# RuyiLian/CheckerPose

Measured on AMD Instinct MI355X. Metric: crops/sec forward (256x256, npt=512), higher is better.
Workload: dtype bf16; 1 GPU; LMO 'ape' hr18GNN2_res6_gnn3Skip_mlpQuery npt=512, PoseNet_GNNskip forward, deterministic random-init weights; global_batch=256, parallelism=dp1 (no forward collective), launch=hipGraph replay of 104 kernel launches

## Files before the change

### checkerpose_amd/csrc/conv3x3_halo.hip

```cpp
#include <stdlib.h>

#include "common.h"
#include <cstring>

struct HaloParams {
  const void* in; const void* w; const float* scale; const float* shift; const void* res; void* out;
  int B, H, W, Cin, in_cs, in_coff, nchunk, Cout, ngroups, NB;
  int tiles_x, tiles_y, total_tiles;
  int act; float slope;
  uint32_t in_bytes, w_bytes;
  long long o_base, o_sb, o_sy, o_sx;
  int Hs, Ws; float up_sy, up_sx;
  const float* seg_w; const float* seg_b; float* seg_out; int seg_S;
};

constexpr int HTH = 8, HTW = 16, HPW = HTW + 2, HPH = HTH + 2, HNPIX = 192;
constexpr int HPLANE = HNPIX * 16, HBUF = 4 * HPLANE;
constexpr int USRH = 7, USRW = 11, USPIX = 80, USBUF = USPIX * 64;

template <typename Tag> struct MmaH;
template <> struct MmaH<F32Tag> {
  static __device__ __forceinline__ void run(const u32x4& w, const u32x4& a, f32x4& acc) {
    acc = __builtin_amdgcn_mfma_f32_16x16x4f32(__uint_as_float(w.x), __uint_as_float(a.x), acc, 0, 0, 0);
    acc = __builtin_amdgcn_mfma_f32_16x16x4f32(__uint_as_float(w.y), __uint_as_float(a.y), acc, 0, 0, 0);
    acc = __builtin_amdgcn_mfma_f32_16x16x4f32(__uint_as_float(w.z), __uint_as_float(a.z), acc, 0, 0, 0);
    acc = __builtin_amdgcn_mfma_f32_16x16x4f32(__uint_as_float(w.w), __uint_as_float(a.w), acc, 0, 0, 0);
  }
};
template <> struct MmaH<BF16Tag> {
  static __device__ __forceinline__ void run(const u32x4& w, const u32x4& a, f32x4& acc) {
    acc = __builtin_amdgcn_mfma_f32_16x16x32_bf16(__builtin_bit_cast(bf16x8, w), __builtin_bit_cast(bf16x8, a), acc, 0, 0, 0);
  }
};

template <typename Tag, bool HAS_RES>
__global__ __launch_bounds__(256) void conv3x3_halo_kernel(const HaloParams p) {
  constexpr int E = Tag::E;
  constexpr int KCH = 4 * E;
  constexpr int ES = 16 / E;
  extern __shared__ __attribute__((aligned(16))) unsigned char smem[];

  const int label = blockIdx.x & 7, slot = blockIdx.x >> 3;
  const int nblk = slot % p.NB;
  const int t = label * ((p.total_tiles + 7) >> 3) + slot / p.NB;
  if (t >= p.total_tiles) return;
  const int tpi = p.tiles_x * p.tiles_y;
  const int b = t / tpi;
  const int trem = t - b * tpi;
  const int ty = trem / p.tiles_x, tx = trem - ty * p.tiles_x;
  const int y0 = ty * HTH, x0 = tx * HTW;

  const int tid = threadIdx.x;
  const int lane = tid & 63;
  const int wave = __builtin_amdgcn_readfirstlane(tid >> 6);
  const int x = lane & 15, q = lane >> 4;
  const int g = nblk * 4 + wave;
  const bool wave_active = g < p.ngroups;

  const __amdgpu_buffer_rsrc_t rsrc = __builtin_amdgcn_make_buffer_rsrc(const_cast<void*>(p.in), 0, p.in_bytes, 0x00020000);
  const __amdgpu_buffer_rsrc_t wrsrc = __builtin_amdgcn_make_buffer_rsrc(const_cast<void*>(p.w), 0, p.w_bytes, 0x00020000);

  uint32_t s_goff[3];
  uint32_t s_lds[3];
  int s_cq[3];
#pragma unroll
  for (int k = 0; k < 3; ++k) {
    const int i = tid + 256 * k;
    const int hp = i >> 2, pq = i & 3;
    const int py = hp / HPW, px = hp - py * HPW;
    const int gy = y0 - 1 + py, gx = x0 - 1 + px;
    const bool ok = (hp < HPH * HPW) & ((unsigned)gy < (unsigned)p.H) & ((unsigned)gx < (unsigned)p.W);
    s_goff[k] = ok ? (uint32_t)(((b * p.H + gy) * p.W + gx) * p.in_cs + p.in_coff + pq * E) : 0xFFFFFFFFu;
    s_lds[k] = (uint32_t)(pq * HPLANE + (hp < HNPIX ? hp : 0) * 16);
    s_cq[k] = pq * E;
  }
  const bool s_do[3] = {true, true, (tid + 512) < HNPIX * 4};

  auto stage_load = [&](u32x4* v, int c) {
    const int c0 = c * KCH;
#pragma unroll
    for (int k = 0; k < 3; ++k) {
      const bool ok = (s_goff[k] != 0xFFFFFFFFu) & (c0 + s_cq[k] < p.Cin);
      const uint32_t off = ok ? (s_goff[k] + (uint32_t)c0) * ES : 0x80000000u;
      v[k] = __builtin_bit_cast(u32x4, __builtin_amdgcn_raw_buffer_load_b128(rsrc, off, 0, 0));
    }
  };
  auto stage_write = [&](const u32x4* v, int buf) {
#pragma unroll
    for (int k = 0; k < 3; ++k)
      if (s_do[k]) *(u32x4*)(smem + buf * HBUF + s_lds[k]) = v[k];
  };

  f32x4 acc[HTH][2];
#pragma unroll
  for (int mt = 0; mt < HTH; ++mt) { acc[mt][0] = f32x4{0.f, 0.f, 0.f, 0.f}; acc[mt][1] = f32x4{0.f, 0.f, 0.f, 0.f}; }

  const uint32_t wbase = ((uint32_t)(wave_active ? g : 0) * p.nchunk * 18u * 64u + lane) * 16u;
  auto w_load = [&](u32x4* w, int c, int tap) {
    const uint32_t off = wbase + ((uint32_t)c * 18u + (uint32_t)tap * 2u) * 1024u;
    w[0] = __builtin_bit_cast(u32x4, __builtin_amdgcn_raw_buffer_load_b128(wrsrc, off, 0, 0));
    w[1] = __builtin_bit_cast(u32x4, __builtin_amdgcn_raw_buffer_load_b128(wrsrc, off + 1024u, 0, 0));
  };
  const uint32_t a_lane = (uint32_t)(q * HPLANE + x * 16);
  auto a_load = [&](u32x4* a, int buf, int tap) {
    const int r = tap / 3, s = tap - 3 * r;
    const unsigned char* base = smem + buf * HBUF + a_lane + (r * HPW + s) * 16;
#pragma unroll
    for (int mt = 0; mt < HTH; ++mt) a[mt] = *(const u32x4*)(base + mt * HPW * 16);
  };
  auto mma = [&](const u32x4* a, const u32x4* w) {
#pragma unroll
    for (int mt = 0; mt < HTH; ++mt) {
      MmaH<Tag>::run(w[0], a[mt], acc[mt][0]);
      MmaH<Tag>::run(w[1], a[mt], acc[mt][1]);
    }
  };

  u32x4 sv[3];
  stage_load(sv, 0);
  u32x4 w0[2], w1[2], w2[2], aA[HTH], aB[HTH];
  w_load(w0, 0, 0);
  w_load(w1, 0, 1);
  stage_write(sv, 0);
  __syncthreads();

#define CP_TAP(T, ACUR, ANEXT, WCUR, WNEXT, CN, TN)                      \
  w_load(WNEXT, CN, TN);                                                 \
  if (T < 8) a_load(ANEXT, buf, T + 1);                                  \
  __builtin_amdgcn_sched_barrier(0);                                     \
  mma(ACUR, WCUR);                                                       \
  __builtin_amdgcn_sched_barrier(0);
  for (int c = 0; c < p.nchunk; ++c) {
    const int buf = c & 1;
    stage_load(sv, c + 1);
    a_load(aA, buf, 0);
    CP_TAP(0, aA, aB, w0, w2, c, 2)
    CP_TAP(1, aB, aA, w1, w0, c, 3)
    CP_TAP(2, aA, aB, w2, w1, c, 4)
    CP_TAP(3, aB, aA, w0, w2, c, 5)
    CP_TAP(4, aA, aB, w1, w0, c, 6)
    CP_TAP(5, aB, aA, w2, w1, c, 7)
    CP_TAP(6, aA, aB, w0, w2, c, 8)
    CP_TAP(7, aB, aA, w1, w0, c + 1, 0)
    CP_TAP(8, aA, aB, w2, w1, c + 1, 1)
    stage_write(sv, buf ^ 1);
    __syncthreads();
  }
#undef CP_TAP

  if (!wave_active) return;
  const int ch = g * 32 + q * 8;
  if (ch >= p.Cout) return;
  const bool hi_ok = ch + 4 < p.Cout;
  const int ox = x0 + x;
  float sc[8], sh[8];
  {
    const f32x4 s0 = *(const f32x4*)(p.scale + ch), t0 = *(const f32x4*)(p.shift + ch);
    const f32x4 s1 = *(const f32x4*)(p.scale + ch + 4), t1 = *(const f32x4*)(p.shift + ch + 4);
#pragma unroll
    for (int j = 0; j < 4; ++j) { sc[j] = s0[j]; sh[j] = t0[j]; sc[4 + j] = s1[j]; sh[4 + j] = t1[j]; }
  }
  if (ox >= p.W) return;
  float rvv[HAS_RES ? HTH : 1][8];
  if constexpr (HAS_RES) {
#pragma unroll
    for (int mt = 0; mt < HTH; ++mt) {
      const int oy = y0 + mt;
#pragma unroll
      for (int j = 0; j < 8; ++j) rvv[mt][j] = 0.f;
      if (oy >= p.H) continue;
      const long long o = p.o_base + (long long)b * p.o_sb + (long long)oy * p.o_sy + (long long)ox * p.o_sx + ch;
      if (E == 4) {
        const f32x4 r0 = *(const f32x4*)((const float*)p.res + o);
#pragma unroll
        for (int j = 0; j < 4; ++j) rvv[mt][j] = r0[j];
        if (hi_ok) {
          const f32x4 r1 = *(const f32x4*)((const float*)p.res + o + 4);
#pragma unroll
          for (int j = 0; j < 4; ++j) rvv[mt][4 + j] = r1[j];
        }
      } else {
        const u32x2 r0 = *(const u32x2*)((const uint16_t*)p.res + o);
        rvv[mt][0] = __uint_as_float(r0.x << 16); rvv[mt][1] = __uint_as_float(r0.x & 0xffff0000u);
        rvv[mt][2] = __uint_as_float(r0.y << 16); rvv[mt][3] = __uint_as_float(r0.y & 0xffff0000u);
        if (hi_ok) {
          const u32x2 r1 = *(const u32x2*)((const uint16_t*)p.res + o + 4);
          rvv[mt][4] = __uint_as_float(r1.x << 16); rvv[mt][5] = __uint_as_float(r1.x & 0xffff0000u);
          rvv[mt][6] = __uint_as_float(r1.y << 16); rvv[mt][7] = __uint_as_float(r1.y & 0xffff0000u);
        }
      }
    }
  }
#pragma unroll
  for (int mt = 0; mt < HTH; ++mt) {
    const int oy = y0 + mt;
    if (oy >= p.H) continue;
    const long long o = p.o_base + (long long)b * p.o_sb + (long long)oy * p.o_sy + (long long)ox * p.o_sx + ch;
    float v[8];
#pragma unroll
    for (int j = 0; j < 4; ++j) { v[j] = acc[mt][0][j] * sc[j] + sh[j]; v[4 + j] = acc[mt][1][j] * sc[4 + j] + sh[4 + j]; }
    if constexpr (HAS_RES) {
#pragma unroll
      for (int j = 0; j < 8; ++j) v[j] += rvv[HAS_RES ? mt : 0][j];
    }
#pragma unroll
    for (int j = 0; j < 8; ++j) {
      v[j] = cp_act_apply(v[j], cp_act_slope(p.act, p.slope));
    }
    if (E == 4) {
      *(f32x4*)((float*)p.out + o) = f32x4{v[0], v[1], v[2], v[3]};
      if (hi_ok) *(f32x4*)((float*)p.out + o + 4) = f32x4{v[4], v[5], v[6], v[7]};
    } else {
      if (hi_ok) {
        u32x4 pk; pk.x = pack_bf16x2(v[0], v[1]); pk.y = pack_bf16x2(v[2], v[3]); pk.z = pack_bf16x2(v[4], v[5]); pk.w = pack_bf16x2(v[6], v[7]);
        if ((((uintptr_t)((uint16_t*)p.out + o)) & 15u) == 0) *(u32x4*)((uint16_t*)p.out + o) = pk;
        else { *(u32x2*)((uint16_t*)p.out + o) = u32x2{pk.x, pk.y}; *(u32x2*)((uint16_t*)p.out + o + 4) = u32x2{pk.z, pk.w}; }
      } else {
        u32x2 pk; pk.x = pack_bf16x2(v[0], v[1]); pk.y = pack_bf16x2(v[2], v[3]);
        *(u32x2*)((uint16_t*)p.out + o) = pk;
      }
    }
  }
}


template <typename Tag, bool HAS_RES, bool UP = false, bool SEG = false>
__global__ __launch_bounds__(256, 2) void conv3x3_halo4_kernel(const HaloParams p) {
  constexpr int E = Tag::E;
  constexpr int KCH = 4 * E;
  constexpr int ES = 16 / E;
  extern __shared__ __attribute__((aligned(16))) unsigned char smem[];
  unsigned char* const sSrc = smem + 2 * HBUF;

  const int label = blockIdx.x & 7, slot = blockIdx.x >> 3;
  const int nblk = slot % p.NB;
  const int t = label * ((p.total_tiles + 7) >> 3) + slot / p.NB;
  if (t >= p.total_tiles) return;
  const int tpi = p.tiles_x * p.tiles_y;
  const int b = t / tpi;
  const int trem = t - b * tpi;
  const int ty = trem / p.tiles_x, tx = trem - ty * p.tiles_x;
  const int y0 = ty * HTH, x0 = tx * HTW;

  const int tid = threadIdx.x;
  const int lane = tid & 63;
  const int wave = __builtin_amdgcn_readfirstlane(tid >> 6);
  const int x = lane & 15, q = lane >> 4;
  const int g = nblk * 4 + wave;

  const __amdgpu_buffer_rsrc_t rsrc = __builtin_amdgcn_make_buffer_rsrc(const_cast<void*>(p.in), 0, p.in_bytes, 0x00020000);
  const __amdgpu_buffer_rsrc_t wrsrc = __builtin_amdgcn_make_buffer_rsrc(const_cast<void*>(p.w), 0, p.w_bytes, 0x00020000);

  uint32_t s_goff[3], s_lds[3];
  int s_cq[3];
#pragma unroll
  for (int k = 0; k < 3; ++k) {
    const int i = tid + 256 * k;
    const int hp = i >> 2, pq = i & 3;
    const int py = hp / HPW, px = hp - py * HPW;
    const int gy = y0 - 1 + py, gx = x0 - 1 + px;
    const bool ok = (hp < HPH * HPW) & ((unsigned)gy < (unsigned)p.H) & ((unsigned)gx < (unsigned)p.W);
    s_goff[k] = ok ? (uint32_t)(((b * p.H + gy) * p.W + gx) * p.in_cs + p.in_coff + pq * E) : 0xFFFFFFFFu;
    s_lds[k] = (uint32_t)(pq * HPLANE + hp * 16);
    s_cq[k] = pq * E;
  }
  auto stage_load = [&](u32x4* v, int c) {
    const int c0 = c * KCH;
#pragma unroll
    for (int k = 0; k < 3; ++k) {
      const bool ok = (s_goff[k] != 0xFFFFFFFFu) & (c0 + s_cq[k] < p.Cin);
      v[k] = __builtin_bit_cast(u32x4, __builtin_amdgcn_raw_buffer_load_b128(rsrc, ok ? (s_goff[k] + (uint32_t)c0) * ES : 0x80000000u, 0, 0));
    }
  };
  auto stage_write = [&](const u32x4* v, int buf) {
#pragma unroll
    for (int k = 0; k < 3; ++k) *(u32x4*)(smem + buf * HBUF + s_lds[k]) = v[k];
  };

  uint32_t u_goff[2], m_off[3];
  float m_lx[3], m_ly[3];
  if constexpr (UP) {
    int sy0, sx0, st_; float fr_;
    cp_up_coord(p.up_sy, y0 > 0 ? y0 - 1 : 0, p.Hs, sy0, st_, fr_);
    cp_up_coord(p.up_sx, x0 > 0 ? x0 - 1 : 0, p.Ws, sx0, st_, fr_);
#pragma unroll
    for (int k = 0; k < 2; ++k) {
      const int i = tid + 256 * k;
      const int sp = i >> 2, pq = i & 3;
      const int ry = sp / USRW, rx = sp - ry * USRW;
      const int yy = sy0 + ry, xx = sx0 + rx;
      const bool ok = (sp < USRH * USRW) & (yy < p.Hs) & (xx < p.Ws);
      u_goff[k] = ok ? (uint32_t)(((b * p.Hs + yy) * p.Ws + xx) * p.in_cs + p.in_coff + pq * E) : 0xFFFFFFFFu;
    }
#pragma unroll
    for (int k = 0; k < 3; ++k) {
      const int i = tid + 256 * k;
      const int hp = i >> 2, pq = i & 3;
      const int py = hp / HPW, px = hp - py * HPW;
      const int gy = y0 - 1 + py, gx = x0 - 1 + px;
      const bool ok = (hp < HPH * HPW) & ((unsigned)gy < (unsigned)p.H) & ((unsigned)gx < (unsigned)p.W);
      int iy0, ix0, my, mx;
      cp_up_coord(p.up_sy, gy, p.Hs, iy0, my, m_ly[k]);
      cp_up_coord(p.up_sx, gx, p.Ws, ix0, mx, m_lx[k]);
      m_off[k] = ok ? (uint32_t)((((iy0 - sy0) * USRW + (ix0 - sx0)) * 4 + pq) * 16) | (uint32_t)(mx | (my << 1) | 4) : 0u;
    }
  }
  auto src_load = [&](u32x4* v, int c) {
    const int c0 = c * KCH;
#pragma unroll
    for (int k = 0; k < 2; ++k) {
      const bool ok = (u_goff[k] != 0xFFFFFFFFu) & (c0 + (tid & 3) * E < p.Cin);
      v[k] = __builtin_bit_cast(u32x4, __builtin_amdgcn_raw_buffer_load_b128(rsrc, ok ? (u_goff[k] + (uint32_t)c0) * ES : 0x80000000u, 0, 0));
    }
  };
  auto src_write = [&](const u32x4* v, int sb) {
    *(u32x4*)(sSrc + sb * USBUF + tid * 16) = v[0];
    if (tid < USPIX * 4 - 256) *(u32x4*)(sSrc + sb * USBUF + (tid + 256) * 16) = v[1];
  };
  auto interp = [&](int k, int sb, int hb) {
    const uint32_t mo = m_off[k];
    const unsigned char* s00 = sSrc + sb * USBUF + (mo & ~15u);
    const uint32_t dx = (mo & 1u) ? 64u : 0u, dy = (mo & 2u) ? (uint32_t)(USRW * 64) : 0u;
    const float lx1 = m_lx[k], lx0 = cp_one_minus(lx1), ly1 = m_ly[k], ly0 = cp_one_minus(ly1);
    const bool in_img = (mo & 4u) != 0u;
    unsigned char* dst = smem + hb * HBUF + s_lds[k];
#pragma unroll
    for (int j = 0; j < 4; ++j) {
      const uint32_t r00 = *(const uint32_t*)(s00 + 4 * j), r01 = *(const uint32_t*)(s00 + dx + 4 * j);
      const uint32_t r10 = *(const uint32_t*)(s00 + dy + 4 * j), r11 = *(const uint32_t*)(s00 + dy + dx + 4 * j);
      uint32_t o;
      if constexpr (E == 4) {
        o = __float_as_uint(cp_bilerp(__uint_as_float(r00), __uint_as_float(r01), __uint_as_float(r10), __uint_as_float(r11), lx0, lx1, ly0, ly1));
      } else {
        const float lo = cp_bilerp(__uint_as_float(r00 << 16), __uint_as_float(r01 << 16), __uint_as_float(r10 << 16), __uint_as_float(r11 << 16), lx0, lx1, ly0, ly1);
        const float hi = cp_bilerp(__uint_as_float(r00 & 0xffff0000u), __uint_as_float(r01 & 0xffff0000u), __uint_as_float(r10 & 0xffff0000u),
                                   __uint_as_float(r11 & 0xffff0000u), lx0, lx1, ly0, ly1);
        o = pack_bf16x2(lo, hi);
      }
      *(uint32_t*)(dst + 4 * j) = in_img ? o : 0u;
    }
  };

  f32x4 acc[HTH][4];
#pragma unroll
  for (int mt = 0; mt < HTH; ++mt)
#pragma unroll
    for (int nt = 0; nt < 4; ++nt) acc[mt][nt] = f32x4{0.f, 0.f, 0.f, 0.f};

  const uint32_t wbase = ((uint32_t)g * p.nchunk * 36u * 64u + lane) * 16u;
  auto w_load = [&](u32x4* w, int c, int tap) {
    const uint32_t off = wbase + ((uint32_t)c * 36u + (uint32_t)tap * 4u) * 1024u;
#pragma unroll
    for (int nt = 0; nt < 4; ++nt) w[nt] = __builtin_bit_cast(u32x4, __builtin_amdgcn_raw_buffer_load_b128(wrsrc, off + nt * 1024u, 0, 0));
  };
  const uint32_t a_lane = (uint32_t)(q * HPLANE + x * 16);
  auto a_load = [&](u32x4* a, int buf, int tap, int half) {
    const int r = tap / 3, s2 = tap - 3 * r;
    const unsigned char* base = smem + buf * HBUF + a_lane + ((r + 4 * half) * HPW + s2) * 16;
#pragma unroll
    for (int i = 0; i < 4; ++i) a[i] = *(const u32x4*)(base + i * HPW * 16);
  };
  auto mma = [&](const u32x4* a, const u32x4* w, int half) {
#pragma unroll
    for (int i = 0; i < 4; ++i)
#pragma unroll
      for (int nt = 0; nt < 4; ++nt) MmaH<Tag>::run(w[nt], a[i], acc[4 * half + i][nt]);
  };

  u32x4 sv[3];
  u32x4 wA[4], wB[4], a0[4], a1[4];
  if constexpr (UP) {
    src_load(sv, 0);
    w_load(wA, 0, 0);
    src_write(sv, 0);
    src_load(sv, 1);
    __syncthreads();
    interp(0, 0, 0); interp(1, 0, 0); interp(2, 0, 0);
    src_write(sv, 1);
  } else {
    stage_load(sv, 0);
    w_load(wA, 0, 0);
    stage_write(sv, 0);
  }
  __syncthreads();

#define CP_TAP4(T, WCUR, WNEXT, CN, TN)                                                 \
  a_load(a1, buf, T, 1); w_load(WNEXT, CN, TN); __builtin_amdgcn_sched_barrier(0);       \
  mma(a0, WCUR, 0); __builtin_amdgcn_sched_barrier(0);                                   \
  if (T < 8) a_load(a0, buf, T + 1, 0);                                                  \
  __builtin_amdgcn_sched_barrier(0);                                                     \
  mma(a1, WCUR, 1); __builtin_amdgcn_sched_barrier(0);
  for (int c = 0; c < p.nchunk; ++c) {
    const int buf = c & 1;
    if constexpr (UP) src_load(sv, c + 2); else stage_load(sv, c + 1);
    a_load(a0, buf, 0, 0);
    CP_TAP4(0, wA, wB, c, 1)
    CP_TAP4(1, wB, wA, c, 2)
    if constexpr (UP) { __builtin_amdgcn_sched_barrier(0); interp(0, buf ^ 1, buf ^ 1); __builtin_amdgcn_sched_barrier(0); }
    CP_TAP4(2, wA, wB, c, 3)
    CP_TAP4(3, wB, wA, c, 4)
    CP_TAP4(4, wA, wB, c, 5)
    if constexpr (UP) { __builtin_amdgcn_sched_barrier(0); interp(1, buf ^ 1, buf ^ 1); __builtin_amdgcn_sched_barrier(0); }
    CP_TAP4(5, wB, wA, c, 6)
    CP_TAP4(6, wA, wB, c, 7)
    CP_TAP4(7, wB, wA, c, 8)
    if constexpr (UP) { __builtin_amdgcn_sched_barrier(0); interp(2, buf ^ 1, buf ^ 1); __builtin_amdgcn_sched_barrier(0); }
    CP_TAP4(8, wA, wB, c + 1, 0)
#pragma unroll
    for (int nt = 0; nt < 4; ++nt) wA[nt] = wB[nt];
    if constexpr (UP) src_write(sv, buf); else stage_write(sv, buf ^ 1);
    __syncthreads();
  }
#undef CP_TAP4

  const int ch = g * 64 + q * 16;
  const int ox = x0 + x;
  if constexpr (!SEG) { if (ox >= p.W) return; }
  const bool xok = SEG ? ox < p.W : true;
  constexpr int SMAX = 2;
  float segw[SEG ? SMAX : 1][16], segp[SEG ? 8 : 1][SEG ? SMAX : 1];
  if constexpr (SEG) {
#pragma unroll
    for (int s_ = 0; s_ < SMAX; ++s_) {
#pragma unroll
      for (int k = 0; k < 4; ++k) {
        const f32x4 w4 = s_ < p.seg_S ? *(const f32x4*)(p.seg_w + (size_t)s_ * p.Cout + ch + 4 * k) : f32x4{0.f, 0.f, 0.f, 0.f};
#pragma unroll
        for (int j = 0; j < 4; ++j) segw[s_][4 * k + j] = w4[j];
      }
#pragma unroll
      for (int mt = 0; mt < 8; ++mt) segp[mt][s_] = 0.f;
    }
  }
  float sc[16], sh[16];
#pragma unroll
  for (int nt = 0; nt < 4; ++nt) {
    const f32x4 s4 = *(const f32x4*)(p.scale + ch + 4 * nt), t4 = *(const f32x4*)(p.shift + ch + 4 * nt);
#pragma unroll
    for (int j = 0; j < 4; ++j) { sc[4 * nt + j] = s4[j]; sh[4 * nt + j] = t4[j]; }
  }
#pragma unroll
  for (int half = 0; half < 2; ++half) {
    u32x4 rr[HAS_RES ? 4 : 1][E == 4 ? 4 : 2];
    if constexpr (HAS_RES) {
#pragma unroll
      for (int i = 0; i < 4; ++i) {
        const int oy = y0 + 4 * half + i;
        const long long o = p.o_base + (long long)b * p.o_sb + (long long)oy * p.o_sy + (long long)ox * p.o_sx + ch;
#pragma unroll
        for (int k = 0; k < (E == 4 ? 4 : 2); ++k) {
          rr[i][k] = u32x4{0u, 0u, 0u, 0u};
          if (oy < p.H) rr[i][k] = E == 4 ? *(const u32x4*)((const float*)p.res + o + 4 * k) : *(const u32x4*)((const uint16_t*)p.res + o + 8 * k);
        }
      }
    }
#pragma unroll
    for (int i = 0; i < 4; ++i) {
      const int mt = 4 * half + i;
      const int oy = y0 + mt;
      if (oy >= p.H) continue;
      const long long o = p.o_base + (long long)b * p.o_sb + (long long)oy * p.o_sy + (long long)ox * p.o_sx + ch;
      float v[16];
#pragma unroll
      for (int nt = 0; nt < 4; ++nt)
#pragma unroll
        for (int j = 0; j < 4; ++j) v[4 * nt + j] = acc[mt][nt][j] * sc[4 * nt + j] + sh[4 * nt + j];
      if constexpr (HAS_RES) {
        if (E == 4) {
#pragma unroll
          for (int k = 0; k < 4; ++k) {
            v[4 * k + 0] += __uint_as_float(rr[i][k].x); v[4 * k + 1] += __uint_as_float(rr[i][k].y);
            v[4 * k + 2] += __uint_as_float(rr[i][k].z); v[4 * k + 3] += __uint_as_float(rr[i][k].w);
          }
        } else {
          float r8[8];
#pragma unroll
          for (int k = 0; k < 2; ++k) {
            Vec16<BF16Tag>::unpack(rr[i][k], r8);
#pragma unroll
            for (int j = 0; j < 8; ++j) v[8 * k + j] += r8[j];
          }
        }
      }
#pragma unroll
      for (int j = 0; j < 16; ++j) {
        v[j] = cp_act_apply(v[j], cp_act_slope(p.act, p.slope));
      }
      if (E == 4) {
        if (xok) {
#pragma unroll
          for (int k = 0; k < 4; ++k) *(f32x4*)((float*)p.out + o + 4 * k) = f32x4{v[4 * k], v[4 * k + 1], v[4 * k + 2], v[4 * k + 3]};
        }
      } else {
        const u32x4 pk0 = Vec16<BF16Tag>::pack(v), pk1 = Vec16<BF16Tag>::pack(v + 8);
        if (xok) {
          *(u32x4*)((uint16_t*)p.out + o) = pk0;
          *(u32x4*)((uint16_t*)p.out + o + 8) = pk1;
        }
        if constexpr (SEG) { Vec16<BF16Tag>::unpack(pk0, v); Vec16<BF16Tag>::unpack(pk1, v + 8); }
      }
      if constexpr (SEG) {
#pragma unroll
        for (int s_ = 0; s_ < SMAX; ++s_) {
          float a = 0.f;
#pragma unroll
          for (int j = 0; j < 16; ++j) a += v[j] * segw[s_][j];
          segp[mt][s_] = a;
        }
      }
    }
  }
  if constexpr (SEG) {
    float* const red = (float*)smem;
#pragma unroll
    for (int mt = 0; mt < 8; ++mt)
#pragma unroll
      for (int s_ = 0; s_ < SMAX; ++s_) {
        float a = segp[mt][s_];
        a += __shfl_xor(a, 16);
        a += __shfl_xor(a, 32);
        if (q == 0) red[((wave * 8 + mt) * 16 + x) * SMAX + s_] = a;
      }
    __syncthreads();
    const int s_ = tid & 1, px = tid >> 1;
    const int mt = px >> 4, xx = px & 15;
    const int oy = y0 + mt, oxx = x0 + xx;
    if (s_ < p.seg_S && oy < p.H && oxx < p.W) {
      float a = p.seg_b[s_];
#pragma unroll
      for (int wv = 0; wv < 4; ++wv) a += red[((wv * 8 + mt) * 16 + xx) * SMAX + s_];
      p.seg_out[(((size_t)b * p.seg_S + s_) * p.H + oy) * p.W + oxx] = a;
    }
  }
}

template <typename Tag>
__global__ void pack_halo4_weight_kernel(const float* __restrict__ w, void* __restrict__ out, int Cout, int Cin, int nchunk,
                                         size_t total) {
  constexpr int E = Tag::E;
  const size_t i = (size_t)blockIdx.x * blockDim.x + threadIdx.x;
  if (i >= total) return;
  const int e = (int)(i % E);
  const int lane = (int)((i / E) % 64);
  size_t blk = i / (E * 64);
  const int nt = (int)(blk % 4); blk /= 4;
  const int tap = (int)(blk % 9); blk /= 9;
  const int c = (int)(blk % nchunk);
  const int g = (int)(blk / nchunk);
  const int row = lane & 15, kq = lane >> 4;
  const int n = g * 64 + (row >> 2) * 16 + nt * 4 + (row & 3);
  const int cin = c * (4 * E) + kq * E + e;
  float v = 0.f;
  if (n < Cout && cin < Cin) v = w[((size_t)n * Cin + cin) * 9 + tap];
  store_elem<Tag>(out, i, v);
}

static inline bool halo_wide(int Cout) { return Cout >= 256 && Cout % 256 == 0 && !cp_knob("CP_NO_HALO4"); }

template <typename Tag, int NT, int KS = 3>
__global__ __launch_bounds__(256) void conv3x3_halo_s_kernel(const HaloParams p) {
  if (KS == 2 && p.seg_S == CP_F16) cp_f16_saturate_on();
  constexpr int E = Tag::E;
  constexpr int KCH = 4 * E;
  constexpr int ES = 16 / E;
  constexpr int NTAP = KS * KS;
  constexpr int WPIECES = NTAP * NT * 64;
  constexpr int WITER = (WPIECES + 255) / 256;
  extern __shared__ __attribute__((aligned(16))) unsigned char smem[];
  unsigned char* const sA = smem;
  unsigned char* const sW = smem + HBUF;

  const int t = blockIdx.x;
  const int tpi = p.tiles_x * p.tiles_y;
  const int b = t / tpi;
  const int trem = t - b * tpi;
  const int ty = trem / p.tiles_x, tx = trem - ty * p.tiles_x;
  const int y0 = ty * HTH, x0 = tx * HTW;

  const int tid = threadIdx.x;
  const int lane = tid & 63;
  const int wave = __builtin_amdgcn_readfirstlane(tid >> 6);
  const int x = lane & 15, q = lane >> 4;

  const __amdgpu_buffer_rsrc_t rsrc = __builtin_amdgcn_make_buffer_rsrc(const_cast<void*>(p.in), 0, p.in_bytes, 0x00020000);
  const __amdgpu_buffer_rsrc_t wrsrc = __builtin_amdgcn_make_buffer_rsrc(const_cast<void*>(p.w), 0, p.w_bytes, 0x00020000);

  uint32_t s_goff[3], s_lds[3];
  int s_cq[3];
#pragma unroll
  for (int k = 0; k < 3; ++k) {
    const int i = tid + 256 * k;
    const int hp = i >> 2, pq = i & 3;
    const int py = hp / HPW, px = hp - py * HPW;
    const int gy = y0 - 1 + py, gx = x0 - 1 + px;
    const bool ok = (hp < HPH * HPW) & ((unsigned)gy < (unsigned)p.H) & ((unsigned)gx < (unsigned)p.W);
    s_goff[k] = ok ? (uint32_t)(((b * p.H + gy) * p.W + gx) * p.in_cs + p.in_coff + pq * E) : 0xFFFFFFFFu;
    s_lds[k] = (uint32_t)(pq * HPLANE + hp * 16);
    s_cq[k] = pq * E;
  }

  f32x4 acc[2][NT];
#pragma unroll
  for (int mt = 0; mt < 2; ++mt)
#pragma unroll
    for (int nt = 0; nt < NT; ++nt) acc[mt][nt] = f32x4{0.f, 0.f, 0.f, 0.f};

  const uint32_t a_lane = (uint32_t)(q * HPLANE + (2 * wave * HPW + x) * 16);
  const int OH = p.H + (3 - KS), OW = p.W + (3 - KS);
  const int ox = x0 + x;
  const int chq = q * 4 * NT;
  long long obase[2];
  bool rok[2];
#pragma unroll
  for (int mt = 0; mt < 2; ++mt) {
    const int oy = y0 + 2 * wave + mt;
    rok[mt] = (oy < OH) & (ox < OW);
    obase[mt] = p.o_base + (long long)b * p.o_sb + (long long)oy * p.o_sy + (long long)ox * p.o_sx + chq;
  }
  f32x4 rv[2][NT];
  if (p.res) {
#pragma unroll
    for (int mt = 0; mt < 2; ++mt)
#pragma unroll
      for (int nt = 0; nt < NT; ++nt) {
        rv[mt][nt] = f32x4{0.f, 0.f, 0.f, 0.f};
        if (rok[mt] && chq + nt * 4 < p.Cout) {
          if (E == 4) rv[mt][nt] = *(const f32x4*)((const float*)p.res + obase[mt] + nt * 4);
          else {
            const u32x2 r2 = *(const u32x2*)((const uint16_t*)p.res + obase[mt] + nt * 4);
            rv[mt][nt] = f32x4{__uint_as_float(r2.x << 16), __uint_as_float(r2.x & 0xffff0000u),
                               __uint_as_float(r2.y << 16), __uint_as_float(r2.y & 0xffff0000u)};
          }
        }
      }
  }
  for (int c = 0; c < p.nchunk; ++c) {
    const int c0 = c * KCH;
    u32x4 sv[3], wv[WITER];
#pragma unroll
    for (int k = 0; k < 3; ++k) {
      const bool ok = (s_goff[k] != 0xFFFFFFFFu) & (c0 + s_cq[k] < p.Cin);
      const uint32_t off = ok ? (s_goff[k] + (uint32_t)c0) * ES : 0x80000000u;
      sv[k] = __builtin_bit_cast(u32x4, __builtin_amdgcn_raw_buffer_load_b128(rsrc, off, 0, 0));
    }
#pragma unroll
    for (int k = 0; k < WITER; ++k) {
      const int i = tid + 256 * k;
      const uint32_t off = i < WPIECES ? ((uint32_t)c * WPIECES + (uint32_t)i) * 16u : 0x80000000u;
      wv[k] = __builtin_bit_cast(u32x4, __builtin_amdgcn_raw_buffer_load_b128(wrsrc, off, 0, 0));
    }
    if (c > 0) __syncthreads();
#pragma unroll
    for (int k = 0; k < 3; ++k) *(u32x4*)(sA + s_lds[k]) = sv[k];
#pragma unroll
    for (int k = 0; k < WITER; ++k) {
      const int i = tid + 256 * k;
      if (i < WPIECES) *(u32x4*)(sW + i * 16) = wv[k];
    }
    __syncthreads();
#pragma unroll
    for (int tap = 0; tap < NTAP; ++tap) {
      const int r = tap / KS, s2 = tap - KS * r;
      const unsigned char* ab = sA + a_lane + (r * HPW + s2) * 16;
      const u32x4 a0 = *(const u32x4*)(ab);
      const u32x4 a1 = *(const u32x4*)(ab + HPW * 16);
#pragma unroll
      for (int nt = 0; nt < NT; ++nt) {
        const u32x4 w = *(const u32x4*)(sW + (tap * NT + nt) * 1024 + lane * 16);
        MmaH<Tag>::run(w, a0, acc[0][nt]);
        MmaH<Tag>::run(w, a1, acc[1][nt]);
      }
    }
  }

  if (ox >= OW) return;
#pragma unroll
  for (int mt = 0; mt < 2; ++mt) {
    if (!rok[mt]) continue;
#pragma unroll
    for (int nt = 0; nt < NT; ++nt) {
      const int ch = chq + nt * 4;
      if (ch >= p.Cout) continue;
      const f32x4 sc = *(const f32x4*)(p.scale + ch), sh = *(const f32x4*)(p.shift + ch);
      float v[4];
#pragma unroll
      for (int j = 0; j < 4; ++j) v[j] = acc[mt][nt][j] * sc[j] + sh[j];
      if (p.res) {
#pragma unroll
        for (int j = 0; j < 4; ++j) v[j] += rv[mt][nt][j];
      }
#pragma unroll
      for (int j = 0; j < 4; ++j) {
        v[j] = cp_act_apply(v[j], cp_act_slope(p.act, p.slope));
      }
      if (E == 4) *(f32x4*)((float*)p.out + obase[mt] + nt * 4) = f32x4{v[0], v[1], v[2], v[3]};
      else if (KS == 2 && p.seg_S == CP_F16) {
        u32x2 pk; pk.x = cp_pack2<true>(v[0], v[1]); pk.y = cp_pack2<true>(v[2], v[3]); *(u32x2*)((uint16_t*)p.out + obase[mt] + nt * 4) = pk;
      }
      else { u32x2 pk; pk.x = pack_bf16x2(v[0], v[1]); pk.y = pack_bf16x2(v[2], v[3]); *(u32x2*)((uint16_t*)p.out + obase[mt] + nt * 4) = pk; }
    }
  }
}

constexpr int FXW = HTW + 4, FXH = HTH + 4, FXPLANE = 256 * 16;

template <typename Tag, int NT>
__global__ __launch_bounds__(256) void basicblock_fused_kernel(const HaloParams p, const void* __restrict__ w2,
                                                               const float* __restrict__ scale2, const float* __restrict__ shift2) {
  constexpr int E = Tag::E;
  constexpr int ES = 16 / E;
  constexpr int WPIECES = 9 * NT * 64;
  constexpr int WITER = (WPIECES + 255) / 256;
  extern __shared__ __attribute__((aligned(16))) unsigned char smem[];
  unsigned char* const sX = smem;
  unsigned char* const sY = smem + 4 * FXPLANE;
  unsigned char* const sW = sY + HBUF;
// ... 714 lines not shown
```

Measured before the change: 25710 crops/s.

## Interleave bf16 upsample interpolation with MFMA taps and pad source LDS pitch

For the bf16 upsample-fused halo conv, bilinear interpolation of the next chunk is split into six half-pixel units. Each unit's LDS loads, lerp math and writes are spread across the MFMA tap sequence using sched_group_barrier, instead of running as three monolithic interp blocks between taps. The source staging buffer row pitch is padded from 64 to 72 bytes to reduce LDS bank conflicts, and the writes now use 8-byte stores. This aims to hide the interpolation VALU and LDS latency under matrix work, at the cost of more register pressure and a more fragile schedule.

```diff
diff --git a/checkerpose_amd/csrc/conv3x3_halo.hip b/checkerpose_amd/csrc/conv3x3_halo.hip
--- a/checkerpose_amd/csrc/conv3x3_halo.hip
+++ b/checkerpose_amd/csrc/conv3x3_halo.hip
@@ -16,7 +16,7 @@
 
 constexpr int HTH = 8, HTW = 16, HPW = HTW + 2, HPH = HTH + 2, HNPIX = 192;
 constexpr int HPLANE = HNPIX * 16, HBUF = 4 * HPLANE;
-constexpr int USRH = 7, USRW = 11, USPIX = 80, USBUF = USPIX * 64;
+constexpr int USRH = 7, USRW = 11, USPIX = 80, USPITCH = 72, USBUF = USPIX * USPITCH;
 
 template <typename Tag> struct MmaH;
 template <> struct MmaH<F32Tag> {
@@ -229,6 +229,7 @@
   constexpr int E = Tag::E;
   constexpr int KCH = 4 * E;
   constexpr int ES = 16 / E;
+  constexpr bool UPS = UP && E != 4;
   extern __shared__ __attribute__((aligned(16))) unsigned char smem[];
   unsigned char* const sSrc = smem + 2 * HBUF;
 
@@ -302,7 +303,7 @@
       int iy0, ix0, my, mx;
       cp_up_coord(p.up_sy, gy, p.Hs, iy0, my, m_ly[k]);
       cp_up_coord(p.up_sx, gx, p.Ws, ix0, mx, m_lx[k]);
-      m_off[k] = ok ? (uint32_t)((((iy0 - sy0) * USRW + (ix0 - sx0)) * 4 + pq) * 16) | (uint32_t)(mx | (my << 1) | 4) : 0u;
+      m_off[k] = ok ? (uint32_t)(((iy0 - sy0) * USRW + (ix0 - sx0)) * USPITCH + pq * 16) | (uint32_t)(mx | (my << 1) | 4) : (uint32_t)(USRH * USRW * USPITCH);
     }
   }
   auto src_load = [&](u32x4* v, int c) {
@@ -314,13 +315,14 @@
     }
   };
   auto src_write = [&](const u32x4* v, int sb) {
-    *(u32x4*)(sSrc + sb * USBUF + tid * 16) = v[0];
-    if (tid < USPIX * 4 - 256) *(u32x4*)(sSrc + sb * USBUF + (tid + 256) * 16) = v[1];
+    unsigned char* d = sSrc + sb * USBUF + (tid >> 2) * USPITCH + (tid & 3) * 16;
+    *(u32x2*)d = u32x2{v[0].x, v[0].y}; *(u32x2*)(d + 8) = u32x2{v[0].z, v[0].w};
+    if (tid < USPIX * 4 - 256) { *(u32x2*)(d + 64 * USPITCH) = u32x2{v[1].x, v[1].y}; *(u32x2*)(d + 64 * USPITCH + 8) = u32x2{v[1].z, v[1].w}; }
   };
   auto interp = [&](int k, int sb, int hb) {
     const uint32_t mo = m_off[k];
-    const unsigned char* s00 = sSrc + sb * USBUF + (mo & ~15u);
-    const uint32_t dx = (mo & 1u) ? 64u : 0u, dy = (mo & 2u) ? (uint32_t)(USRW * 64) : 0u;
+    const unsigned char* s00 = sSrc + sb * USBUF + (mo & ~7u);
+    const uint32_t dx = (mo & 1u) ? (uint32_t)USPITCH : 0u, dy = (mo & 2u) ? (uint32_t)(USRW * USPITCH) : 0u;
     const float lx1 = m_lx[k], lx0 = cp_one_minus(lx1), ly1 = m_ly[k], ly0 = cp_one_minus(ly1);
     const bool in_img = (mo & 4u) != 0u;
     unsigned char* dst = smem + hb * HBUF + s_lds[k];
@@ -328,17 +330,43 @@
     for (int j = 0; j < 4; ++j) {
       const uint32_t r00 = *(const uint32_t*)(s00 + 4 * j), r01 = *(const uint32_t*)(s00 + dx + 4 * j);
       const uint32_t r10 = *(const uint32_t*)(s00 + dy + 4 * j), r11 = *(const uint32_t*)(s00 + dy + dx + 4 * j);
-      uint32_t o;
-      if constexpr (E == 4) {
-        o = __float_as_uint(cp_bilerp(__uint_as_float(r00), __uint_as_float(r01), __uint_as_float(r10), __uint_as_float(r11), lx0, lx1, ly0, ly1));
-      } else {
-        const float lo = cp_bilerp(__uint_as_float(r00 << 16), __uint_as_float(r01 << 16), __uint_as_float(r10 << 16), __uint_as_float(r11 << 16), lx0, lx1, ly0, ly1);
-        const float hi = cp_bilerp(__uint_as_float(r00 & 0xffff0000u), __uint_as_float(r01 & 0xffff0000u), __uint_as_float(r10 & 0xffff0000u),
-                                   __uint_as_float(r11 & 0xffff0000u), lx0, lx1, ly0, ly1);
-        o = pack_bf16x2(lo, hi);
-      }
+      const uint32_t o = __float_as_uint(cp_bilerp(__uint_as_float(r00), __uint_as_float(r01), __uint_as_float(r10), __uint_as_float(r11), lx0, lx1, ly0, ly1));
       *(uint32_t*)(dst + 4 * j) = in_img ? o : 0u;
     }
+  };
+  auto up_issue = [&](int u, int sb, u32x2* cr) {
+    const uint32_t mo = m_off[u >> 1];
+    const unsigned char* s00 = sSrc + sb * USBUF + (mo & ~7u) + 8 * (u & 1);
+    const uint32_t dx = (mo & 1u) ? (uint32_t)USPITCH : 0u, dy = (mo & 2u) ? (uint32_t)(USRW * USPITCH) : 0u;
+    cr[0] = *(const u32x2*)s00; cr[1] = *(const u32x2*)(s00 + dx);
+    cr[2] = *(const u32x2*)(s00 + dy); cr[3] = *(const u32x2*)(s00 + dy + dx);
+  };
+  auto up_lerp = [&](int u, int j, const u32x2* cr) -> uint32_t {
+    const int k = u >> 1;
+    const float lx1 = m_lx[k], lx0 = cp_one_minus(lx1), ly1 = m_ly[k], ly0 = cp_one_minus(ly1);
+    const uint32_t r00 = cr[0][j], r01 = cr[1][j], r10 = cr[2][j], r11 = cr[3][j];
+    if constexpr (E == 4) {
+      return __float_as_uint(cp_bilerp(__uint_as_float(r00), __uint_as_float(r01), __uint_as_float(r10), __uint_as_float(r11), lx0, lx1, ly0, ly1));
+    } else {
+      const float lo = cp_bilerp(__uint_as_float(r00 << 16), __uint_as_float(r01 << 16), __uint_as_float(r10 << 16), __uint_as_float(r11 << 16), lx0, lx1, ly0, ly1);
+      const float hi = cp_bilerp(__uint_as_float(r00 & 0xffff0000u), __uint_as_float(r01 & 0xffff0000u), __uint_as_float(r10 & 0xffff0000u),
+                                 __uint_as_float(r11 & 0xffff0000u), lx0, lx1, ly0, ly1);
+      float hi_ = hi; asm("" : "+v"(hi_));
+      return pack_bf16x2(lo, hi_);
+    }
+  };
+  auto up_write = [&](int u, int hb, uint32_t o0, uint32_t o1) {
+    *(u32x2*)(smem + hb * HBUF + s_lds[u >> 1] + 8 * (u & 1)) = u32x2{o0, o1};
+  };
+  auto up_sched = [&](bool write) {
+#pragma unroll
+    for (int i = 0; i < 8; ++i) {
+      __builtin_amdgcn_sched_group_barrier(0x8, 1, 0);
+      __builtin_amdgcn_sched_group_barrier(0x2, 2, 0);
+      __builtin_amdgcn_sched_group_barrier(0x8, 1, 0);
+      __builtin_amdgcn_sched_group_barrier(0x2, 1, 0);
+    }
+    if (write) __builtin_amdgcn_sched_group_barrier(0x200, 1, 0);
   };
 
   f32x4 acc[HTH][4];
@@ -369,13 +397,24 @@
 
   u32x4 sv[3];
   u32x4 wA[4], wB[4], a0[4], a1[4];
+  u32x2 cr[4];
+  uint32_t up_o0 = 0u;
   if constexpr (UP) {
     src_load(sv, 0);
     w_load(wA, 0, 0);
     src_write(sv, 0);
     src_load(sv, 1);
     __syncthreads();
-    interp(0, 0, 0); interp(1, 0, 0); interp(2, 0, 0);
+#pragma unroll
+    for (int h = 0; h < 2; ++h) {
+      if constexpr (UPS) {
+        u32x2 cp[3][4];
+#pragma unroll
+        for (int u = 3 * h; u < 3 * h + 3; ++u) up_issue(u, 0, cp[u - 3 * h]);
+#pragma unroll
+        for (int u = 3 * h; u < 3 * h + 3; ++u) up_write(u, 0, up_lerp(u, 0, cp[u - 3 * h]), up_lerp(u, 1, cp[u - 3 * h]));
+      } else if (h == 0) { interp(0, 0, 0); interp(1, 0, 0); interp(2, 0, 0); }
+    }
     src_write(sv, 1);
   } else {
     stage_load(sv, 0);
@@ -384,27 +423,35 @@
   }
   __syncthreads();
 
+#define CP_UP_ISSUE(G) if constexpr (UPS && (G) % 3 == 0) up_issue((G) / 3, buf ^ 1, cr);
+#define CP_UP_LERP(G)                                                                                            \
+  if constexpr (UPS && (G) % 3 == 1) { up_o0 = up_lerp((G) / 3, 0, cr); up_sched(false); }                       \
+  if constexpr (UPS && (G) % 3 == 2) { up_write((G) / 3, buf ^ 1, up_o0, up_lerp((G) / 3, 1, cr)); up_sched(true); }
 #define CP_TAP4(T, WCUR, WNEXT, CN, TN)                                                 \
-  a_load(a1, buf, T, 1); w_load(WNEXT, CN, TN); __builtin_amdgcn_sched_barrier(0);       \
-  mma(a0, WCUR, 0); __builtin_amdgcn_sched_barrier(0);                                   \
+  a_load(a1, buf, T, 1); w_load(WNEXT, CN, TN); CP_UP_ISSUE(2 * T)                       \
+  __builtin_amdgcn_sched_barrier(0);                                                     \
+  mma(a0, WCUR, 0); CP_UP_LERP(2 * T) __builtin_amdgcn_sched_barrier(0);                 \
   if (T < 8) a_load(a0, buf, T + 1, 0);                                                  \
+  CP_UP_ISSUE(2 * T + 1)                                                                 \
   __builtin_amdgcn_sched_barrier(0);                                                     \
-  mma(a1, WCUR, 1); __builtin_amdgcn_sched_barrier(0);
+  mma(a1, WCUR, 1); CP_UP_LERP(2 * T + 1) __builtin_amdgcn_sched_barrier(0);             \
+  if constexpr (UP && !UPS && (T == 1 || T == 4 || T == 7)) { interp(T / 3, buf ^ 1, buf ^ 1); __builtin_amdgcn_sched_barrier(0); }
   for (int c = 0; c < p.nchunk; ++c) {
     const int buf = c & 1;
-    if constexpr (UP) src_load(sv, c + 2); else stage_load(sv, c + 1);
+    if constexpr (UP) {
+#pragma unroll
+      for (int k = 0; k < 3; ++k) asm volatile("" : "+v"(m_off[k]), "+v"(m_lx[k]), "+v"(m_ly[k]));
+      src_load(sv, c + 2);
+    } else stage_load(sv, c + 1);
     a_load(a0, buf, 0, 0);
     CP_TAP4(0, wA, wB, c, 1)
     CP_TAP4(1, wB, wA, c, 2)
-    if constexpr (UP) { __builtin_amdgcn_sched_barrier(0); interp(0, buf ^ 1, buf ^ 1); __builtin_amdgcn_sched_barrier(0); }
     CP_TAP4(2, wA, wB, c, 3)
     CP_TAP4(3, wB, wA, c, 4)
     CP_TAP4(4, wA, wB, c, 5)
-    if constexpr (UP) { __builtin_amdgcn_sched_barrier(0); interp(1, buf ^ 1, buf ^ 1); __builtin_amdgcn_sched_barrier(0); }
     CP_TAP4(5, wB, wA, c, 6)
     CP_TAP4(6, wA, wB, c, 7)
     CP_TAP4(7, wB, wA, c, 8)
-    if constexpr (UP) { __builtin_amdgcn_sched_barrier(0); interp(2, buf ^ 1, buf ^ 1); __builtin_amdgcn_sched_barrier(0); }
     CP_TAP4(8, wA, wB, c + 1, 0)
 #pragma unroll
     for (int nt = 0; nt < 4; ++nt) wA[nt] = wB[nt];
@@ -412,6 +459,8 @@
     __syncthreads();
   }
 #undef CP_TAP4
+#undef CP_UP_ISSUE
+#undef CP_UP_LERP
 
   const int ch = g * 64 + q * 16;
   const int ox = x0 + x;
```

After: 25940 crops/s, median of 6. Within noise of the previous version (+0.9%).
